# IN2-ViAUn/Exploration-of-Potential

Hardware: AMD Instinct MI355X
Metric: training images/sec, YOLOX-l 24p 640x640 bf16 (higher is better)
Workload: dtype bf16; 1 GPU; YOLOX-l-24p (CSPDarknet53+PAFPN+24p head) train step, 640x640, batch 20/GPU, 10 GTs/img, SimOTA + 24-circle GIoU loss, SGD nesterov; global_batch=20, parallelism=dp1, hip_graph=forward and backward as two lanes of captured segments, loss, update

## Files before the change

exploration-of-potential_amd/csrc/conv_igemm.hip:

```cpp
#include <stdlib.h>
#include <type_traits>
#include <atomic>
#include "igemm.h"

using namespace ep24_igemm;

namespace {

constexpr int KOPT_TILED = 1, KOPT_NARROW_EPI = 2, KOPT_PER_CLASS = 4;
constexpr int KOPT_REMOVED = 16 | 32 | 64;
constexpr int KOPT_NO_DEEP = 128;
constexpr int KOPT_TILED256 = 256;
constexpr int KOPT_NO_WREG = 512;
constexpr int KOPT_PATCH8 = 8;

template <int BN, bool OUT_F32, int EPI, int NSTG = 2>
__device__ __forceinline__ void igemm_dma_tile(const IgemmArgs& p, const int tile_m, const int tile_n) {
    constexpr int WN = BN / 64, WM = 4 / WN, MT = BM / WM / 16, NT = 4;
    constexpr int A_BYTES = BM * 128, B_BYTES = BN * 128, STAGE = A_BYTES + B_BYTES;
    constexpr int A_INSTR = BM * 8 / 64 / 4;
    constexpr int B_INSTR = BN * 8 / 64 / 4;
    extern __shared__ __attribute__((aligned(16))) char smem[];

    const int tid = threadIdx.x, lane = tid & 63, wave = __builtin_amdgcn_readfirstlane(tid >> 6);
// ... 7 lines not shown
    const auto src_rsrc = __builtin_amdgcn_make_buffer_rsrc(const_cast<bf16*>(p.src), 0, p.src_bytes, 0x00020000);
    const auto wt_rsrc = __builtin_amdgcn_make_buffer_rsrc(const_cast<bf16*>(p.wt), 0, p.wt_bytes, 0x00020000);
    int rowoff[A_INSTR];
    unsigned vmask[A_INSTR];
    int iy0v[A_INSTR], ix0v[A_INSTR];
#pragma unroll
    for (int i = 0; i < A_INSTR; ++i) {
        const long m = m0 + (wave * A_INSTR + i) * 8 + (lane >> 3);
        const bool rv = m < p.M;
        const int mm = rv ? (int)m : 0;
        const int n = fdiv(mm, p.d_plane);
        const int rem = mm - n * (p.GH * p.GW);
        const int gy = fdiv(rem, p.d_gw), gx = rem - gy * p.GW;
        const int iy0 = gy * p.sy, ix0 = gx * p.sx;
        rowoff[i] = (int)((((long)n * p.SH * p.SW + (long)iy0 * p.SW + ix0) * p.ld_src + lchunk * 8) * 2);
        iy0v[i] = rv ? iy0 : -(1 << 20);
        ix0v[i] = ix0;
        vmask[i] = 0u;
    }
    const unsigned long long tdy = p.tap_dy, tdx = p.tap_dx, tsl = p.tap_slot;
    for (int t = 0; t < p.T; ++t) {
        const int dy = (int)((tdy >> (4 * t)) & 15ull) - 8, dx = (int)((tdx >> (4 * t)) & 15ull) - 8;
#pragma unroll
        for (int i = 0; i < A_INSTR; ++i) {
            const int iy = iy0v[i] + dy, ix = ix0v[i] + dx;
            if (iy >= 0 && iy < p.SH && ix >= 0 && ix < p.SW) vmask[i] |= 1u << t;
        }
    }
    const int ld2 = (int)p.ld_src * 2;
    int wvoff[B_INSTR];
#pragma unroll
    for (int i = 0; i < B_INSTR; ++i) {
        const int q = (wave * B_INSTR + i) * 8 + (lane >> 3);
        const int r = (q & ~63) + ((q & 15) << 2) + ((q >> 4) & 3);
        wvoff[i] = n0 + r < p.N ? (int)((((long)(n0 + r) * p.WT * p.K) + lchunk * 8) * 2) : OOB;
    }
    const int kmax = (p.K - lchunk * 8 + BK - 1) / BK;
    const int ktail = (p.K & (BK - 1)) ? KC - 1 : KC;

    int is_t = 0, is_kc = 0;
    auto issue = [&](int buf) {
        const int t = is_t, kc = is_kc;
        if (++is_t == p.T) { is_t = 0; ++is_kc; }
        const bool tail = kc >= ktail;
        const int ktm = tail ? -(int)(kc < kmax) : -1;
        const int dy = (int)((tdy >> (4 * t)) & 15ull) - 8, dx = (int)((tdx >> (4 * t)) & 15ull) - 8;
        const int a_s = (dy * p.SW + dx) * ld2 + kc * (BK * 2);
        const unsigned b_s = (unsigned)(((int)((tsl >> (4 * t)) & 15ull) * p.K + kc * BK) * 2);
        char* stage = smem + buf * STAGE;
#pragma unroll
        for (int i = 0; i < A_INSTR; ++i) {
            const int m = -(int)((vmask[i] >> t) & 1u) & ktm;
            const int vo = ((rowoff[i] + a_s) & m) | (OOB & ~m);
            __builtin_amdgcn_raw_ptr_buffer_load_lds(src_rsrc, (lptr_t)(stage + (wave * A_INSTR + i) * 1024), 16, vo, 0, 0, 0);
        }
#pragma unroll
        for (int i = 0; i < B_INSTR; ++i) {
            const int v = (int)((unsigned)wvoff[i] + b_s);
            const int vo = (v & ktm) | (OOB & ~ktm);
            __builtin_amdgcn_raw_ptr_buffer_load_lds(wt_rsrc, (lptr_t)(stage + A_BYTES + (wave * B_INSTR + i) * 1024), 16, vo, 0, 0, 0);
        }
    };

    f32x4 acc[MT][NT];
#pragma unroll
    for (int i = 0; i < MT; ++i)
#pragma unroll
// ... 13 lines not shown
                fb[q] = *reinterpret_cast<const bf16x8*>(lb + swz(wn * 64 + q * 16 + frow, ks * 4 + fq));
#pragma unroll
            for (int i = 0; i < MT; ++i)
#pragma unroll
                for (int q = 0; q < NT; ++q)
                    acc[i][q] = __builtin_amdgcn_mfma_f32_16x16x32_bf16(fa[i], fb[q], acc[i][q], 0, 0, 0);
        }
    };
    if constexpr (NSTG >= 3) {
#pragma unroll
        for (int i = 0; i < NSTG - 1; ++i)
            if (i < n_iter) issue(i);
        int st = 0;
        for (int it = 0; it < n_iter; ++it) {
            const int ahead = n_iter - 1 - it;
            if (NSTG >= 4 && ahead >= 2) asm volatile("s_waitcnt vmcnt(%0)" ::"n"(2 * (A_INSTR + B_INSTR)) : "memory");
            else if (ahead >= 1) asm volatile("s_waitcnt vmcnt(%0)" ::"n"(A_INSTR + B_INSTR) : "memory");
            else asm volatile("s_waitcnt vmcnt(0)" ::: "memory");
            __builtin_amdgcn_s_barrier();
            asm volatile("" ::: "memory");
            if (it + NSTG - 1 < n_iter) issue(st == 0 ? NSTG - 1 : st - 1);
            compute(smem + st * STAGE);
            st = st == NSTG - 1 ? 0 : st + 1;
        }
    } else {
    issue(0);
    for (int it = 0; it < n_iter; ++it) {
        __syncthreads();
        if (it + 1 < n_iter) issue((it + 1) & 1);
        compute(smem + (it & 1) * STAGE);
    }
    }

    igemm_epilogue<BN, OUT_F32, MT, EPI>(p, acc, m0, n0, tile_m, smem);
}

template <int BN, bool OUT_F32, int EPI, int NSTG = 2>
__device__ __forceinline__ void igemm_dma_body(const IgemmArgs& p, const int bid, const int nwg) {
    const int xcd = bid & 7, qq = nwg >> 3, rr = nwg & 7;
    const int tile_id = (xcd < rr ? xcd * (qq + 1) : rr * (qq + 1) + (xcd - rr) * qq) + (bid >> 3);
    const int tiles_n = (p.N + BN - 1) / BN;
    const int tile_m = tile_id / tiles_n;
    igemm_dma_tile<BN, OUT_F32, EPI, NSTG>(p, tile_m, tile_id - tile_m * tiles_n);
}

template <int BN, bool OUT_F32, int EPI = 0>
__global__ __launch_bounds__(256) void igemm_dma_kernel(const IgemmArgs p) {
    igemm_dma_body<BN, OUT_F32, EPI>(p, (int)blockIdx.x, (int)gridDim.x);
}

#ifndef EP24_DEEP_STAGES
#define EP24_DEEP_STAGES 3
#endif
template <int EPI>
__global__ __launch_bounds__(256) void igemm_dma_deep_kernel(const IgemmArgs p) {
    igemm_dma_body<128, false, EPI, EP24_DEEP_STAGES>(p, (int)blockIdx.x, (int)gridDim.x);
}

struct IgemmMulti {
    IgemmArgs a;
    int T[4];
    unsigned long long tap_dy[4], tap_dx[4], tap_slot[4];
    int dy0[4], dx0[4];
    int prefix[5];
    int n;
};

template <int BN>
__global__ __launch_bounds__(256) void igemm_dma_multi_kernel(const IgemmMulti q) {
    int cls = 0;
#pragma unroll
    for (int c = 1; c < 4; ++c)
        if (c < q.n && (int)blockIdx.x >= q.prefix[c]) cls = c;
    cls = __builtin_amdgcn_readfirstlane(cls);
    IgemmArgs p = q.a;
    p.T = q.T[cls];
    p.tap_dy = q.tap_dy[cls]; p.tap_dx = q.tap_dx[cls]; p.tap_slot = q.tap_slot[cls];
    p.dy0 = q.dy0[cls]; p.dx0 = q.dx0[cls];
    igemm_dma_body<BN, false, 1>(p, (int)blockIdx.x - q.prefix[cls], q.prefix[cls + 1] - q.prefix[cls]);
}

template <int BN, int H, int EPI, int NKS, bool ACC, bool GATHER = false, int XF = 0, bool BNR = false>
__global__ __launch_bounds__(256, XF == 3 ? 3 : 2) void igemm_stream_kernel(const IgemmArgs p, int bpn) {
    constexpr int SP = BN / 64, NTW = SP * 4, MT = XF ? 1 : 2, XS = XF ? 2 : 1, RG = 128;
    static_assert(XF == 0 || XF == 4 || H == 1, "the transformed-A forms make one K pass");
    static_assert(!BNR || (EPI == 0 && !GATHER && XF == 4), "the fused reduce belongs to the plain input-gradient form in 16-row blocks (with the transformed-A form it doubled that form's VALU work and spilled: measured, not kept)");
    constexpr int OOB = 0x7FFFFFF0;
    constexpr bool XAUX = XF >= 2;
    constexpr int XNC = XF == 3 ? 5 : XF == 4 ? 0 : 2;
    constexpr int XKP = H * 128;
    constexpr int XC_FLOATS = XF ? XNC * XKP : 0;
    static_assert(XF == 0 || (EPI == 0 && !GATHER), "the transformed-A forms are training forms of the plain 1x1 kernel");
    constexpr int NPAN_ = (H - 1) * 2 + (NKS + 1) / 2;
    extern __shared__ __attribute__((aligned(16))) char smem[];
    const int tid = threadIdx.x, lane = tid & 63, wave = __builtin_amdgcn_readfirstlane(tid >> 6);
    const int frow = lane & 15, fq = lane >> 4;
    const int n_tiles = (p.N + BN - 1) / BN;
    const int xcd = blockIdx.x & 7, rest = blockIdx.x >> 3;
    const int nt = rest % n_tiles, rb = GATHER ? xcd * (bpn >> 3) + rest / n_tiles : (rest / n_tiles) * 8 + xcd;
    const int n0 = nt * BN;

    const auto rsrc = __builtin_amdgcn_make_buffer_rsrc(const_cast<bf16*>(p.src), 0, p.src_bytes, 0x00020000);
    const auto drsrc = __builtin_amdgcn_make_buffer_rsrc(p.dst, 0, p.dst_bytes, 0x00020000);
    const long n_groups = (p.M + RG - 1) / RG;
    const long my_groups = rb < n_groups ? (n_groups - rb + bpn - 1) / bpn : 0;
    const long units = my_groups * H * XS;

    typedef int v4i __attribute__((ext_vector_type(4)));
    typedef unsigned v2u __attribute__((ext_vector_type(2)));
    int gdy[GATHER ? NKS : 1], gdx[GATHER ? NKS : 1], gof[GATHER ? NKS : 1];
    if constexpr (GATHER) {
#pragma unroll
// ... 426 lines not shown
    constexpr int NPAN = (H - 1) * 2 + (NKS + 1) / 2;
    size_t lds = (size_t)NPAN * BN * 128 + (size_t)(XF == 3 ? 5 * H * 128 : (XF == 1 || XF == 2) ? 2 * H * 128 : 0) * sizeof(float) + (size_t)(BNR ? 4 * BN : 0) * sizeof(float);
    if (lds < 4096) lds = 4096;
    const dim3 grid((unsigned)(bpn * n_tiles));
    if constexpr (XF == 3 || BNR) {
        if (a.accumulate) hipLaunchKernelGGL((igemm_stream_kernel<BN, H, 0, NKS, true, false, XF, BNR>), grid, dim3(256), lds, stream, a, (int)bpn);
        else hipLaunchKernelGGL((igemm_stream_kernel<BN, H, 0, NKS, false, false, XF, BNR>), grid, dim3(256), lds, stream, a, (int)bpn);
    } else if constexpr (XF != 0) {
        hipLaunchKernelGGL((igemm_stream_kernel<BN, H, 0, NKS, false, false, XF>), grid, dim3(256), lds, stream, a, (int)bpn);
    } else if constexpr (GATHER) {
        if (a.epi_infer) hipLaunchKernelGGL((igemm_stream_kernel<BN, H, 2, NKS, false, true>), grid, dim3(256), lds, stream, a, (int)bpn);
        else hipLaunchKernelGGL((igemm_stream_kernel<BN, H, 0, NKS, false, true>), grid, dim3(256), lds, stream, a, (int)bpn);
    } else {
        if (a.epi_infer) hipLaunchKernelGGL((igemm_stream_kernel<BN, H, 2, NKS, false>), grid, dim3(256), lds, stream, a, (int)bpn);
        else if (a.accumulate) hipLaunchKernelGGL((igemm_stream_kernel<BN, H, 1, NKS, true>), grid, dim3(256), lds, stream, a, (int)bpn);
        else if (!a.stats) hipLaunchKernelGGL((igemm_stream_kernel<BN, H, 1, NKS, false>), grid, dim3(256), lds, stream, a, (int)bpn);
        else hipLaunchKernelGGL((igemm_stream_kernel<BN, H, 0, NKS, false>), grid, dim3(256), lds, stream, a, (int)bpn);
    }
}

template <int XF>
void launch_stream_xf(const IgemmArgs& a, hipStream_t stream) {
    if (a.N > 64) { if (a.K > 64) launch_stream<128, 1, 4, false, XF>(a, stream); else launch_stream<128, 1, 2, false, XF>(a, stream); }
    else          { if (a.K > 64) launch_stream<64, 1, 4, false, XF>(a, stream); else launch_stream<64, 1, 2, false, XF>(a, stream); }
}

void launch_stream_bnr(const IgemmArgs& a, hipStream_t stream) {
    if (a.N > 64) { if (a.K > 128) launch_stream<128, 2, 4, false, 4, true>(a, stream); else if (a.K > 64) launch_stream<128, 1, 4, false, 4, true>(a, stream); else launch_stream<128, 1, 2, false, 4, true>(a, stream); }
    else          { if (a.K > 128) launch_stream<64, 2, 4, false, 4, true>(a, stream); else if (a.K > 64) launch_stream<64, 1, 4, false, 4, true>(a, stream); else launch_stream<64, 1, 2, false, 4, true>(a, stream); }
}

bool xf_shape_ok(long M, int K, int N) { return K > 0 && K % 8 == 0 && K <= 128 && N > 0 && N % 4 == 0 && N <= 128 && M > 0; }

template <int BN, bool F32>
void launch_variant(const IgemmArgs& a, unsigned tiles, hipStream_t stream) {
    constexpr size_t lds = 2 * (BM * 128 + BN * 128);
    if (a.epi_infer && !F32) hipLaunchKernelGGL((igemm_dma_kernel<BN, false, 2>), dim3(tiles), dim3(256), lds, stream, a);
    else if (!a.stats && !F32) hipLaunchKernelGGL((igemm_dma_kernel<BN, false, 1>), dim3(tiles), dim3(256), lds, stream, a);
    else hipLaunchKernelGGL((igemm_dma_kernel<BN, F32>), dim3(tiles), dim3(256), lds, stream, a);
}

int check_extents(const IgemmArgs& a) {
    for (int t = 0; t < a.T; ++t)
        EP24_REQUIRE(a.T <= 16 && a.oy[t] >= -8 && a.oy[t] <= 7 && a.ox[t] >= -8 && a.ox[t] <= 7 && a.wslot[t] >= 0 && a.wslot[t] <= 15, EP24_E_UNSUPPORTED,
                     "conv: tap %d (offset %d, %d, weight slot %d) does not fit the packed tap tables (offsets -8 .. 7, slots 0 .. 15)", t, a.oy[t], a.ox[t], a.wslot[t]);
    const long src_b = (((long)a.B * a.SH * a.SW - 1) * a.ld_src + a.K) * 2;
    const long wt_b = (long)a.N * a.WT * a.K * 2;
    EP24_REQUIRE(src_b < 0x7FFF0000L && wt_b < 0x7FFF0000L && a.M < (1L << 31) && (long)a.B * a.SH * a.SW < (1L << 31), EP24_E_UNSUPPORTED,
                 "conv: a source of %ld bytes / weights of %ld bytes / %ld output pixels are beyond what the 32-bit tile addressing covers "
                 "(2 GiB per operand): split the batch", src_b, wt_b, (long)a.M);
    return EP24_OK;
}

void prepare(IgemmArgs& a, int kernel_opts) {
    a.narrow_epi = (kernel_opts & KOPT_NARROW_EPI) ? 1 : 0;
    a.src_bytes = (unsigned)((((long)a.B * a.SH * a.SW - 1) * a.ld_src + a.K) * 2);
    a.wt_bytes = (unsigned)((long)a.N * a.WT * a.K * 2);
    a.d_plane = make_fastdiv((unsigned)(a.GH * a.GW)); a.d_gw = make_fastdiv((unsigned)a.GW);
    a.tap_dy = a.tap_dx = a.tap_slot = 0ull;
    for (int t = 0; t < a.T; ++t) {
        a.toff[t] = (int)(((long)a.oy[t] * a.SW + a.ox[t]) * a.ld_src * 2);
        a.tap_dy |= (unsigned long long)((a.oy[t] + 8) & 15) << (4 * t);
        a.tap_dx |= (unsigned long long)((a.ox[t] + 8) & 15) << (4 * t);
        a.tap_slot |= (unsigned long long)(a.wslot[t] & 15) << (4 * t);
    }
}

int launch_multi(IgemmArgs* cls, int n, hipStream_t stream, int kernel_opts) {
    IgemmMulti q{};
    q.n = n;
    bool wide = true;
    for (int i = 0; i < n; ++i) {
        if (int rc = check_extents(cls[i])) return rc;
        prepare(cls[i], kernel_opts);
        {
            const IgemmArgs& c = cls[i];
            const long ext = (((long)(c.B - 1) * c.dbs + c.dp0 + (long)((c.GH - 1) * c.dsy + c.dy0) * c.DW + (c.GW - 1) * c.dsx + c.dx0) * c.ld_dst + c.N) * 2;
            cls[i].dst_bytes = (ext > 0 && ext < 0x7FFF0000L) ? (unsigned)ext : 0u;
        }
        wide = wide && cls[i].N > 64 && (long)ep24_cdiv(cls[i].M, BM) * ep24_cdiv(cls[i].N, 128) > 256;
        const IgemmArgs &x = cls[i], &y = cls[0];
        EP24_REQUIRE(x.src == y.src && x.ld_src == y.ld_src && x.B == y.B && x.SH == y.SH && x.SW == y.SW && x.GH == y.GH && x.GW == y.GW && x.sy == y.sy &&
                     x.sx == y.sx && x.wt == y.wt && x.WT == y.WT && x.K == y.K && x.N == y.N && x.dst == y.dst && x.ld_dst == y.ld_dst && x.DH == y.DH &&
                     x.DW == y.DW && x.dsy == y.dsy && x.dsx == y.dsx && x.dbs == y.dbs && x.dp0 == y.dp0 && x.accumulate == y.accumulate && x.M == y.M &&
                     !x.bias && !x.stats && !x.bnr_z && !x.epi_infer, EP24_E_ARG, "conv_igemm_multi: the classes of one launch share everything but their taps and parity");
    }
    q.a = cls[0];
    for (int i = 1; i < n; ++i) q.a.dst_bytes = (q.a.dst_bytes && cls[i].dst_bytes) ? std::max(q.a.dst_bytes, cls[i].dst_bytes) : 0u;
    for (int i = 0; i < n; ++i) {
        q.T[i] = cls[i].T; q.tap_dy[i] = cls[i].tap_dy; q.tap_dx[i] = cls[i].tap_dx; q.tap_slot[i] = cls[i].tap_slot;
        q.dy0[i] = cls[i].dy0; q.dx0[i] = cls[i].dx0;
        q.prefix[i + 1] = q.prefix[i] + ep24_cdiv(cls[i].M, BM) * ep24_cdiv(cls[i].N, wide ? 128 : 64);
    }
    const unsigned blocks = (unsigned)q.prefix[n];
    const dim3 grid(blocks);
    if (wide) hipLaunchKernelGGL((igemm_dma_multi_kernel<128>), grid, dim3(256), 2 * (BM * 128 + 128 * 128), stream, q);
    else hipLaunchKernelGGL((igemm_dma_multi_kernel<64>), grid, dim3(256), 2 * (BM * 128 + 64 * 128), stream, q);
    EP24_LAUNCH_CHECK("ep24_conv_igemm_multi");
    return EP24_OK;
}

int launch(IgemmArgs a, bool out_f32, hipStream_t stream, int kernel_opts = 0, bool dry = false, int* kernel_id = nullptr) {
    EP24_REQUIRE(!(kernel_opts & KOPT_REMOVED), EP24_E_UNSUPPORTED,
                 "conv: kernel_opts bits 4 - 6 selected variants that were measured, lost and removed; their source is at commit 6cc7180");
    if (!dry) { if (int rc = check_extents(a)) return rc; }
    prepare(a, kernel_opts);
    const bool plain_dst = a.dsy == 1 && a.dsx == 1 && a.dy0 == 0 && a.dx0 == 0 && a.DW == a.GW && a.dp0 == 0 && a.dbs == (long)a.GH * a.GW;
    const long dst_b = ((a.M - 1) * a.ld_dst + a.N) * 2;
    const long dst_ext = plain_dst ? dst_b : (((long)(a.B - 1) * a.dbs + a.dp0 + (long)((a.GH - 1) * a.dsy + a.dy0) * a.DW + (a.GW - 1) * a.dsx + a.dx0) * a.ld_dst + a.N) * 2;
    a.dst_bytes = (!out_f32 && dst_ext > 0 && dst_ext < 0x7FFF0000L) ? (unsigned)dst_ext : 0u;
    const bool stream_ok = a.T == 1 && a.sy == 1 && a.sx == 1 && a.oy[0] == 0 && a.ox[0] == 0 && a.GH == a.SH && a.GW == a.SW &&
                           (a.K <= 128 || (a.K <= 256 && (a.M >= 100000 || !(kernel_opts & KOPT_TILED256)))) && !out_f32 && (!a.bias || a.epi_infer) && plain_dst &&
                           a.ld_dst % 4 == 0 && a.N % 4 == 0 && dst_b < 0x7FFF0000L;
    if (a.bnr_z && !stream_ok) {
        EP24_REQUIRE(plain_dst && !out_f32 && !a.accumulate && !a.narrow_epi && !a.bias && !a.epi_infer && a.N % 8 == 0 && a.ld_dst % 8 == 0 &&
                     a.bnr_ldz % 8 == 0 && ((reinterpret_cast<unsigned long long>(a.dst) | reinterpret_cast<unsigned long long>(a.bnr_z)) & 15) == 0 &&
                     a.bnr_reps > 0, EP24_E_ARG, "conv_dgrad_bnr: needs a plain, first-writer bf16 destination with channel counts / strides in multiples of 8");
    }
    if (stream_ok) {
        if (dry) { *kernel_id = 2; return EP24_OK; }
        a.dst_bytes = (unsigned)dst_b;
        if (a.bnr_z) {
            const long z_b = ((a.M - 1) * a.bnr_ldz + a.N) * 2;
            EP24_REQUIRE(!a.stats && !a.epi_infer && a.bnr_reps > 0 && a.bnr_ldz % 4 == 0 && z_b < 0x7FFF0000L && a.bnr_act == 1, EP24_E_ARG,
                         "conv_dgrad_bnr (1x1): an input gradient of a SiLU unit, z rows 8-byte aligned, operands below 2 GiB");
            a.bnr_z_bytes = (unsigned)z_b;
            launch_stream_bnr(a, stream);
            EP24_LAUNCH_CHECK("ep24_conv_igemm_stream_bnr");
            return EP24_OK;
// ... 7 lines not shown
                            (!a.epi_res || ((a.epi_ldres & 3) == 0 && (reinterpret_cast<unsigned long long>(a.epi_res) & 7) == 0));
    if (a.T == 9 && a.sy == 1 && a.sx == 1 && a.GH == a.SH && a.GW == a.SW && plain_dst && !out_f32 && ((!a.bias && !a.epi_infer) || infer_ring) &&
        !(kernel_opts & KOPT_TILED)) {
        int prc = EP24_OK;
        if (!a.epi_infer && !(kernel_opts & KOPT_NO_WREG) && launch_wreg(a, stream, dry, &prc)) {
            if (dry) { *kernel_id = 6; return EP24_OK; }
            if (prc) return prc;
            EP24_LAUNCH_CHECK("ep24_conv_wreg");
            return EP24_OK;
        }
        if (!(kernel_opts & KOPT_PATCH8) && launch_ring(a, stream, dry, &prc)) {
            if (dry) { *kernel_id = 3; return EP24_OK; }
            if (prc) return prc;
            EP24_LAUNCH_CHECK("ep24_conv_ring");
            return EP24_OK;
        }
        if (!a.epi_infer && launch_patch(a, stream, dry, &prc)) {
            if (dry) { *kernel_id = 1; return EP24_OK; }
            if (prc) return prc;
            EP24_LAUNCH_CHECK("ep24_conv_patch");
            return EP24_OK;
        }
    }
    if (dry) { *kernel_id = 0; return EP24_OK; }
    const bool wide = a.N > 64 && (long)ep24_cdiv(a.M, BM) * ep24_cdiv(a.N, 128) > 256;
    if (!wide && a.N > 64 && !out_f32 && !a.epi_infer && !(kernel_opts & KOPT_NO_DEEP) && a.T * ep24_cdiv(a.K, BK) >= 8) {
        static std::atomic<unsigned long long> done{0};
        int dev = 0;
        EP24_REQUIRE(hipGetDevice(&dev) == hipSuccess, EP24_E_LAUNCH, "conv: hipGetDevice failed");
        const unsigned long long bit = 1ull << (dev & 63);
        if (!(done.load(std::memory_order_acquire) & bit)) {
            hipError_t e = hipFuncSetAttribute((const void*)igemm_dma_deep_kernel<0>, hipFuncAttributeMaxDynamicSharedMemorySize, 160 * 1024);
            if (e == hipSuccess) e = hipFuncSetAttribute((const void*)igemm_dma_deep_kernel<1>, hipFuncAttributeMaxDynamicSharedMemorySize, 160 * 1024);
            EP24_REQUIRE(e == hipSuccess, EP24_E_LAUNCH, "conv: hipFuncSetAttribute(MaxDynamicSharedMemorySize) failed on device %d: %s", dev, hipGetErrorString(e));
            done.fetch_or(bit, std::memory_order_release);
        }
        const unsigned t128 = (unsigned)ep24_cdiv(a.M, BM) * (unsigned)ep24_cdiv(a.N, 128);
        if (a.stats) hipLaunchKernelGGL(igemm_dma_deep_kernel<0>, dim3(t128), dim3(256), EP24_DEEP_STAGES * (BM * 128 + 128 * 128), stream, a);
        else hipLaunchKernelGGL(igemm_dma_deep_kernel<1>, dim3(t128), dim3(256), EP24_DEEP_STAGES * (BM * 128 + 128 * 128), stream, a);
        EP24_LAUNCH_CHECK("ep24_conv_igemm_deep");
        return EP24_OK;
    }
    const unsigned tiles = (unsigned)ep24_cdiv(a.M, BM) * (unsigned)ep24_cdiv(a.N, wide ? 128 : 64);
    if (wide) {
        if (out_f32) launch_variant<128, true>(a, tiles, stream);
        else launch_variant<128, false>(a, tiles, stream);
    } else {
        if (out_f32) launch_variant<64, true>(a, tiles, stream);
        else launch_variant<64, false>(a, tiles, stream);
    }
    EP24_LAUNCH_CHECK("ep24_conv_igemm");
    return EP24_OK;
}

}

static int conv_fwd_impl(const void* x, int64_t ld_x, const void* w, void* y, int64_t ld_y, int y_f32,
                         int64_t y_batch_rows, int64_t y_row0, const float* bias, int64_t* stats,
                         int stats_replicas, int B, int H, int W, int Cin, int Cout, int ksize, int stride,
                         int kernel_opts, void* stream, bool dry = false, int* kernel_id = nullptr) {
    EP24_REQUIRE(dry || (x && w && y), EP24_E_ARG, "conv_fwd: null pointer");
    EP24_REQUIRE(Cin % 8 == 0 && Cin > 0, EP24_E_ARG, "conv_fwd: Cin=%d must be a multiple of 8", Cin);
    EP24_REQUIRE((ksize == 1 || ksize == 3) && (stride == 1 || stride == 2), EP24_E_UNSUPPORTED,
                 "conv_fwd: k=%d s=%d unsupported", ksize, stride);
    EP24_REQUIRE(ld_x % 8 == 0 && (y_f32 || ld_y % 4 == 0), EP24_E_ARG, "conv_fwd: ld_x %% 8 / ld_y %% 4 alignment");
    EP24_REQUIRE(!stats || stats_replicas > 0, EP24_E_ARG, "conv_fwd: stats_replicas");
    const int pad = (ksize - 1) / 2;
    const int OH = (H + 2 * pad - ksize) / stride + 1, OW = (W + 2 * pad - ksize) / stride + 1;
    IgemmArgs a{};
    a.src = (const bf16*)x; a.ld_src = ld_x; a.B = B; a.SH = H; a.SW = W;
    a.GH = OH; a.GW = OW; a.sy = stride; a.sx = stride;
// ... 269 lines not shown
```

exploration-of-potential_amd/csrc/conv_ring.hip:

```cpp
#include <atomic>
#include <type_traits>
#include "igemm.h"

using namespace ep24_igemm;

namespace {

typedef unsigned v4u __attribute__((ext_vector_type(4)));

constexpr int NCW = 4, NLW = 4;
constexpr int NS = 3;
constexpr int RBN = 128, RBM = 256;
constexpr int B_BYTES = RBN * 128;
constexpr int B_INSTR = RBN / 8 / NLW;
constexpr int MT = 8, NT = 4;
constexpr int ZB = 128;
constexpr int LA = 8;
constexpr int SPIN_LIMIT = 1 << 14;

__device__ unsigned g_ring_timeouts;

#ifdef EP24_STAMPS
__device__ unsigned long long g_ring_stamps[64 * 8];
__device__ unsigned long long g_ring_estamps[64 * 8];
// ... 204 lines not shown
__device__ __forceinline__ void ring_store_half(const IgemmArgs& p, long m0, int n0, char* smem) {
    typedef int v4i_ __attribute__((ext_vector_type(4)));
    constexpr int T = ALL ? (NCW + NLW) * 64 : NLW * 64, NK = 4 * 64 * 8 / T;
    const int t = ALL ? (int)threadIdx.x : (int)threadIdx.x - NCW * 64;
    const auto drs = __builtin_amdgcn_make_buffer_rsrc(reinterpret_cast<bf16*>(p.dst), 0, p.dst_bytes, 0x00020000);
    const int rt = t >> 3, ch = t & 7;
    const char* lsrc = smem + HALF * 8192 + rt * 128 + ((ch ^ (rt & 7)) << 4);
    const int ld2 = (int)p.ld_dst * 2;
    const long mt = m0 + HALF * 64 + rt;
    const int cc0 = n0 + ch * 8;
    const int off_t = (int)((mt * p.ld_dst + cc0) * 2);
    bf16x8 v_[NK];
    int off[NK];
#pragma unroll
    for (int k = 0; k < NK; ++k) {
        const int area = ALL ? k : k >> 1, rr = ALL ? 0 : (k & 1) * 32;
        v_[k] = *reinterpret_cast<const bf16x8*>(lsrc + area * 16384 + rr * 128);
        const int dm = (area >> 1) * 128 + rr, dc = (area & 1) * 64;
        off[k] = (mt + dm < p.M && cc0 + dc < p.N) ? off_t + dm * ld2 + dc * 2 : OOB;
    }
    if (p.accumulate) {
        bf16x8 o_[NK];
#pragma unroll
        for (int k = 0; k < NK; ++k) o_[k] = __builtin_bit_cast(bf16x8, __builtin_amdgcn_raw_buffer_load_b128(drs, off[k], 0, 0));
#pragma unroll
        for (int k = 0; k < NK; ++k)
#pragma unroll
            for (int e = 0; e < 8; ++e) v_[k][e] = (bf16)((float)v_[k][e] + (float)o_[k][e]);
    }
#pragma unroll
    for (int k = 0; k < NK; ++k) __builtin_amdgcn_raw_buffer_store_b128(__builtin_bit_cast(v4i_, v_[k]), drs, off[k], 0, 0);
}

template <int PPS, int EMODE>
__global__ __launch_bounds__((NCW + NLW) * 64) void conv_ring_kernel(const IgemmArgs p, const int NP, const int halo, const int npb) {
    extern __shared__ __attribute__((aligned(16))) char smem[];
    const int tid = threadIdx.x, lane = tid & 63, wave = __builtin_amdgcn_readfirstlane(tid >> 6);
    const int nwg = gridDim.x, xcd = blockIdx.x & 7, qq = nwg >> 3, rr = nwg & 7;
    const int tile_id = (xcd < rr ? xcd * (qq + 1) : rr * (qq + 1) + (xcd - rr) * qq) + (blockIdx.x >> 3);
    const int tiles_n = (p.N + RBN - 1) / RBN;
    const int tile_m = tile_id / tiles_n;
    const long m0 = (long)tile_m * RBM;
    const int n0 = (tile_id - tile_m * tiles_n) * RBN;
    const int KC = (p.K + BK - 1) / BK;
    const int PBYTES = NP * 1024;
    const int bb = npb * PBYTES;
    unsigned* const flags = reinterpret_cast<unsigned*>(smem + ZB + bb + NS * B_BYTES);
    lds_u32* const f_full = (lds_u32*)(lptr_t)flags;
    lds_u32* const f_free = f_full + 4;
    lds_u32* const f_err = f_full + 8;
    const int sgn = p.oy[0] < 0 ? 1 : -1;

    if (reinterpret_cast<unsigned long>((lptr_t)smem) != 0ul) {
        if (tid == 0) atomicAdd(&g_ring_timeouts, 1u << 16);
        return;
    }
    if (tid < 12) flags[tid] = 0u;
    if (tid >= 64 && tid < 64 + ZB / 4) reinterpret_cast<unsigned*>(smem)[tid - 64] = 0u;
    __syncthreads();

    const bool wide = !p.narrow_epi && (p.N & 7) == 0 && (p.ld_dst & 7) == 0 && (reinterpret_cast<unsigned long long>(p.dst) & 15) == 0;

    f32x4 acc[MT][NT];
#pragma unroll
    for (int i = 0; i < MT; ++i)
#pragma unroll
        for (int q = 0; q < NT; ++q) acc[i][q] = (f32x4){0.f, 0.f, 0.f, 0.f};
#ifdef EP24_STAMPS
    unsigned long long st_t0 = 0, st_r0 = 0, st_t1 = 0, st_t2 = 0, st_spin = 0;
    unsigned st_nspin = 0;
#endif

    auto loader_main = [&]() {
        const int lw = wave - NCW;
        const int lchunk = (lane & 7) ^ ((lane >> 3) & 7);
        const auto src_rsrc = __builtin_amdgcn_make_buffer_rsrc(const_cast<bf16*>(p.src), 0, p.src_bytes, 0x00020000);
        const auto wt_rsrc = __builtin_amdgcn_make_buffer_rsrc(const_cast<bf16*>(p.wt), 0, p.wt_bytes, 0x00020000);
        const int kmax = (p.K - lchunk * 8 + BK - 1) / BK;
        const int ktail = (p.K & (BK - 1)) ? KC - 1 : KC;
        const int NPW = (NP + NLW - 1) / NLW;
        const unsigned msrc = (unsigned)((long)p.B * p.SH * p.SW);
        const int prow0 = (int)(m0 - halo) + (lane >> 3);
        const int ld2 = (int)p.ld_src * 2;
        const unsigned pv0 = (unsigned)prow0 * (unsigned)ld2 + lchunk * 16;
        auto issue_patch = [&](int pbuf_off, int kc, int i) {
            int g = (i < NPW ? i : NPW - 1) * NLW + lw;
            g = g < NP ? g : NP - 1;
            const unsigned ps = (unsigned)(prow0 + 8 * g);
            bool ok = ps < msrc;
            if (kc >= ktail) ok = ok && kc < kmax;
            const int vo = ok ? (int)(pv0 + (unsigned)(8 * g * ld2 + kc * (BK * 2))) : OOB;
            __builtin_amdgcn_raw_ptr_buffer_load_lds(src_rsrc, (lptr_t)(smem + ZB + pbuf_off + g * 1024), 16, vo, 0, 0, 0);
        };
        int wvoff[B_INSTR];
#pragma unroll
        for (int i = 0; i < B_INSTR; ++i) {
            const int q = (lw * B_INSTR + i) * 8 + (lane >> 3);
            const int r = (q & ~63) + ((q & 15) << 2) + ((q >> 4) & 3);
            wvoff[i] = n0 + r < p.N ? (int)((((long)(n0 + r) * p.WT * p.K) + lchunk * 8) * 2) : OOB;
        }
        auto issue_b = [&](int stage, int t, int kc) {
            const int b_s = (t * p.K + kc * BK) * 2;
#pragma unroll
            for (int i = 0; i < B_INSTR; ++i) {
                int vo = wvoff[i] == OOB ? OOB : wvoff[i] + b_s;
                if (kc >= ktail) vo = kc < kmax ? vo : OOB;
                __builtin_amdgcn_raw_ptr_buffer_load_lds(wt_rsrc, (lptr_t)(smem + ZB + bb + stage * B_BYTES + (lw * B_INSTR + i) * 1024), 16, vo, 0, 0, 0);
            }
        };
        for (int i = 0; i < NPW; ++i) issue_patch(0, 0, i);
        unsigned j = 0;
        for (int kc = 0; kc < KC; ++kc) {
            const int pnext = ((kc + 1) & 1) * PBYTES;
            const bool more = kc + 1 < KC;
#pragma unroll 1
            for (int ty = 0; ty < 3; ++ty) {
                auto step = [&](auto txc) {
                    constexpr int tx = decltype(txc)::value;
                    const int t = ty * 3 + tx;
                    if (j >= (unsigned)NS) spin_until(f_free, j - (NS - 1), f_err);
                    issue_b(tx, t, kc);
                    const bool slice = more && t >= 2;
                    if (slice) {
#pragma unroll
                        for (int i = 0; i < PPS; ++i) issue_patch(pnext, kc + 1, (t - 2) * PPS + i);
                        wait_vmcnt_c<PPS>();
                    } else {
                        wait_vmcnt_c<0>();
                    }
                    ++j;
                    if (lane == 0) st_flag(f_full + lw, j);
// ... 125 lines not shown
                    }
                    if constexpr (g < LA) mma_row(g % MT, pa[g], g < MT ? fb0 : fb1);
                    else mma_row(g % MT, F[g], g < MT ? fb0 : fb1);
                    if constexpr (g >= 9 - LA && g < 9 - LA + MT) {
                        constexpr int i = g - (9 - LA);
                        ra[i] = row_addr(tan, i, tn);
                        pin(ra[i]);
                    }
                    __builtin_amdgcn_sched_barrier(0);
                };
                group(std::integral_constant<int, 0>{}); group(std::integral_constant<int, 1>{});
                group(std::integral_constant<int, 2>{}); group(std::integral_constant<int, 3>{});
                group(std::integral_constant<int, 4>{}); group(std::integral_constant<int, 5>{});
                group(std::integral_constant<int, 6>{}); group(std::integral_constant<int, 7>{});
                group(std::integral_constant<int, 8>{}); group(std::integral_constant<int, 9>{});
                group(std::integral_constant<int, 10>{}); group(std::integral_constant<int, 11>{});
                group(std::integral_constant<int, 12>{}); group(std::integral_constant<int, 13>{});
                group(std::integral_constant<int, 14>{}); group(std::integral_constant<int, 15>{});
                ++j;
            };
            tap_step(std::integral_constant<int, 0>{});
            tap_step(std::integral_constant<int, 1>{});
            tap_step(std::integral_constant<int, 2>{});
        }
    }
#ifdef EP24_STAMPS
    st_t2 = STAMP();
#endif
    };

    const bool consumer = wave < NCW;
    if (consumer) consumer_main(); else loader_main();
    mfma_drain();
    if (wide) ring_epilogue<EMODE>(p, acc, consumer, m0, n0, tile_m, smem);
    else if (consumer) igemm_epilogue<RBN, false, MT, 0, NCW, false>(p, acc, m0, n0, tile_m, smem);
    else return;
    const int cw = wave; (void)cw;
#ifdef EP24_STAMPS
    if (blockIdx.x < 32 && lane == 0 && (cw == 0 || cw == NCW - 1)) {
        unsigned long long* o = g_ring_stamps + (blockIdx.x * 2 + (cw != 0)) * 8;
        o[0] = st_t1 - st_t0; o[1] = st_t2 - st_t1; o[2] = STAMP() - st_t2; o[3] = st_spin; o[4] = st_nspin;
        o[5] = __builtin_amdgcn_s_memrealtime() - st_r0; o[6] = STAMP() - st_t0; o[7] = 9 * KC;
    }
#endif
}

template <int PPS, int EMODE>
int launch_ring_pps(const IgemmArgs& a, int NP, int halo, int npb, size_t lds, hipStream_t stream) {
    const unsigned tiles = (unsigned)ep24_cdiv(a.M, RBM) * (unsigned)ep24_cdiv(a.N, RBN);
    static std::atomic<unsigned long long> done{0};
    int dev = 0;
    EP24_REQUIRE(hipGetDevice(&dev) == hipSuccess, EP24_E_LAUNCH, "conv_ring: hipGetDevice failed");
    const unsigned long long bit = 1ull << (dev & 63);
    if (!(done.load(std::memory_order_acquire) & bit)) {
        const hipError_t e = hipFuncSetAttribute((const void*)conv_ring_kernel<PPS, EMODE>, hipFuncAttributeMaxDynamicSharedMemorySize, 160 * 1024);
        EP24_REQUIRE(e == hipSuccess, EP24_E_LAUNCH, "conv_ring: hipFuncSetAttribute(MaxDynamicSharedMemorySize, 160 KB) failed on device %d: %s", dev,
                     hipGetErrorString(e));
        done.fetch_or(bit, std::memory_order_release);
    }
    IgemmArgs b = a;
    const long dst_b = ((a.M - 1) * a.ld_dst + a.N) * 2;
    EP24_REQUIRE(dst_b < 0x7FFF0000L, EP24_E_UNSUPPORTED, "conv_ring: a destination of %ld bytes is beyond the 32-bit offsets of its stores (launch_ring sends such a layer to the tiled kernel)", dst_b);
    b.dst_bytes = (unsigned)dst_b;
    hipLaunchKernelGGL((conv_ring_kernel<PPS, EMODE>), dim3(tiles), dim3((NCW + NLW) * 64), lds, stream, b, NP, halo, npb);
    return EP24_OK;
}

}

namespace ep24_igemm { int bn_barrier_timeouts(); }

extern "C" int ep24_conv_ring_timeouts(void) {
    unsigned v = 0;
    if (hipMemcpyFromSymbol(&v, HIP_SYMBOL(g_ring_timeouts), sizeof(v)) != hipSuccess) return -1;
    const int bb = ep24_igemm::bn_barrier_timeouts();
    return bb < 0 ? -1 : (int)v + bb;
}

#ifdef EP24_STAMPS
extern "C" int ep24_debug_read_ring_stamps(unsigned long long* host, int n) {
    return hipMemcpyFromSymbol(host, HIP_SYMBOL(g_ring_stamps), sizeof(unsigned long long) * (size_t)n) == hipSuccess ? 0 : -1;
}
extern "C" int ep24_debug_read_ring_estamps(unsigned long long* host, int n) {
    return hipMemcpyFromSymbol(host, HIP_SYMBOL(g_ring_estamps), sizeof(unsigned long long) * (size_t)n) == hipSuccess ? 0 : -1;
}
#endif

namespace ep24_igemm {

bool launch_ring(const IgemmArgs& a, hipStream_t stream, bool dry, int* rc) {
    const int sgn = a.oy[0] < 0 ? 1 : -1;
    for (int t = 0; t < 9; ++t)
        if (a.oy[t] != sgn * (t / 3 - 1) || a.ox[t] != sgn * (t % 3 - 1) || a.wslot[t] != t) return false;
    if (a.K % 8 != 0) return false;
    if (a.bnr_z) return false;
    if (((a.M - 1) * a.ld_dst + a.N) * 2 >= 0x7FFF0000L) return false;
    if (a.N <= 64 || (long)ep24_cdiv(a.M, RBM) * ep24_cdiv(a.N, RBN) < 200) return false;
    const int halo = a.SW + 1;
    const int npb = a.K > BK ? 2 : 1;
    const int np = (RBM + 2 * halo + 7) / 8;
    const size_t lds = ZB + (size_t)npb * np * 1024 + NS * (size_t)B_BYTES + 64;
    const int npw = (np + NLW - 1) / NLW;
    if (lds > 160 * 1024 || npw > 7 * 3) return false;
    if ((size_t)npb * np * 1024 + NS * (size_t)B_BYTES < (size_t)NCW * MT * 16 * 128) return false;
    if (!dry) {
        const int pps = (npw + 6) / 7;
        if (a.epi_infer)
            *rc = pps <= 1 ? launch_ring_pps<1, 1>(a, np, halo, npb, lds, stream)
                : pps == 2 ? launch_ring_pps<2, 1>(a, np, halo, npb, lds, stream)
                           : launch_ring_pps<3, 1>(a, np, halo, npb, lds, stream);
        else if (a.stats)
            *rc = pps <= 1 ? launch_ring_pps<1, 0>(a, np, halo, npb, lds, stream)
                : pps == 2 ? launch_ring_pps<2, 0>(a, np, halo, npb, lds, stream)
                           : launch_ring_pps<3, 0>(a, np, halo, npb, lds, stream);
        else
            *rc = pps <= 1 ? launch_ring_pps<1, 2>(a, np, halo, npb, lds, stream)
                : pps == 2 ? launch_ring_pps<2, 2>(a, np, halo, npb, lds, stream)
                           : launch_ring_pps<3, 2>(a, np, halo, npb, lds, stream);
    }
    return true;
}

}
```

exploration-of-potential_amd/csrc/igemm.h:

```cpp
#pragma once
#include "common.h"

namespace ep24_igemm {

struct IgemmArgs {
    const bf16* src; long ld_src; int B, SH, SW;
    int GH, GW, sy, sx;
    int T; int oy[16]; int ox[16]; int wslot[16];
    const bf16* wt; int WT; int K; int N;
    void* dst; long ld_dst; int DH, DW, dsy, dsx, dy0, dx0; long dbs, dp0;
    int accumulate;
    const float* bias;
    long long* stats; int stats_replicas;
    int epi_act; const bf16* epi_res; long epi_ldres; int epi_infer;
    int toff[16];
    unsigned long long tap_dy, tap_dx, tap_slot;
    unsigned src_bytes, wt_bytes;
    unsigned dst_bytes;
    FastDiv d_plane, d_gw;
    long M;
    int narrow_epi;
    const bf16* bnr_z; long bnr_ldz; const float* bnr_mean; const float* bnr_invstd; const float* bnr_gamma; const float* bnr_beta;
    long long* bnr_dgamma; long long* bnr_dbeta; long bnr_rep_stride; int bnr_reps; int bnr_act;
    unsigned bnr_z_bytes;
// ... 229 lines not shown
        const float bv = fq == 0 ? b4[0] : fq == 1 ? b4[1] : fq == 2 ? b4[2] : b4[3];
        const int c = n0 + wn * 64 + 4 * frow + fq;
        long long* st = p.stats + (long)(tile_m % p.stats_replicas) * 2 * p.N;
        if (c < p.N) {
            atomicAdd((unsigned long long*)(st + c), (unsigned long long)to_fix(av));
            atomicAdd((unsigned long long*)(st + (long)p.N + c), (unsigned long long)to_fix(bv));
        }
    } else if (STATS && p.stats) {
        __syncthreads();
        float* red = reinterpret_cast<float*>(smem);
#pragma unroll
        for (int q = 0; q < 4; ++q) {
            float a = s1[q], b = s2[q];
            a += __shfl_xor(a, 16, 64); a += __shfl_xor(a, 32, 64);
            b += __shfl_xor(b, 16, 64); b += __shfl_xor(b, 32, 64);
            if (fq == 0) {
                red[(wave * 2 + 0) * 64 + 4 * frow + q] = a;
                red[(wave * 2 + 1) * 64 + 4 * frow + q] = b;
            }
        }
        __syncthreads();
        long long* st = p.stats + (long)(tile_m % p.stats_replicas) * 2 * p.N;
        for (int i = tid; i < 2 * BN; i += NWV * 64) {
            const int which = i / BN, c = i - which * BN;
            const int wcol = c >> 6;
            float v = 0.f;
#pragma unroll
            for (int r = 0; r < WM; ++r) v += red[((r * WN + wcol) * 2 + which) * 64 + (c & 63)];
            if (n0 + c < p.N) atomicAdd((unsigned long long*)(st + (long)which * p.N + n0 + c), (unsigned long long)to_fix(v));
        }
    }
}

bool launch_patch(const IgemmArgs& a, hipStream_t stream, bool dry, int* rc);
bool launch_ring(const IgemmArgs& a, hipStream_t stream, bool dry, int* rc);
bool launch_wreg(const IgemmArgs& a, hipStream_t stream, bool dry, int* rc);

}
```

Measured before the change: 1027 images/s.

## Store conv outputs directly from registers by permuting weight rows

After: 1035 images/s (median of 6 runs). About the same (+0.7%).

```diff
diff --git a/exploration-of-potential_amd/csrc/conv_igemm.hip b/exploration-of-potential_amd/csrc/conv_igemm.hip
--- a/exploration-of-potential_amd/csrc/conv_igemm.hip
+++ b/exploration-of-potential_amd/csrc/conv_igemm.hip
@@ -63,7 +63,8 @@
 #pragma unroll
     for (int i = 0; i < B_INSTR; ++i) {
         const int q = (wave * B_INSTR + i) * 8 + (lane >> 3);
-        const int r = (q & ~63) + ((q & 15) << 2) + ((q >> 4) & 3);
+        const int r = EPI == 3 ? (q & ~63) + ((q & 7) << 3) + ((q & 8) >> 1) + ((q >> 4) & 3)
+                               : (q & ~63) + ((q & 15) << 2) + ((q >> 4) & 3);
         wvoff[i] = n0 + r < p.N ? (int)((((long)(n0 + r) * p.WT * p.K) + lchunk * 8) * 2) : OOB;
     }
     const int kmax = (p.K - lchunk * 8 + BK - 1) / BK;
@@ -143,7 +144,8 @@
     }
     }
 
-    igemm_epilogue<BN, OUT_F32, MT, EPI>(p, acc, m0, n0, tile_m, smem);
+    if constexpr (EPI == 3) igemm_store_direct<MT, WN>(p, acc, m0, n0);
+    else igemm_epilogue<BN, OUT_F32, MT, EPI>(p, acc, m0, n0, tile_m, smem);
 }
 
 template <int BN, bool OUT_F32, int EPI, int NSTG = 2>
@@ -177,7 +179,7 @@
     int n;
 };
 
-template <int BN>
+template <int BN, int EPI = 1>
 __global__ __launch_bounds__(256) void igemm_dma_multi_kernel(const IgemmMulti q) {
     int cls = 0;
 #pragma unroll
@@ -188,7 +190,7 @@
     p.T = q.T[cls];
     p.tap_dy = q.tap_dy[cls]; p.tap_dx = q.tap_dx[cls]; p.tap_slot = q.tap_slot[cls];
     p.dy0 = q.dy0[cls]; p.dx0 = q.dx0[cls];
-    igemm_dma_body<BN, false, 1>(p, (int)blockIdx.x - q.prefix[cls], q.prefix[cls + 1] - q.prefix[cls]);
+    igemm_dma_body<BN, false, EPI>(p, (int)blockIdx.x - q.prefix[cls], q.prefix[cls + 1] - q.prefix[cls]);
 }
 
 template <int BN, int H, int EPI, int NKS, bool ACC, bool GATHER = false, int XF = 0, bool BNR = false>
@@ -681,10 +683,16 @@
 
 bool xf_shape_ok(long M, int K, int N) { return K > 0 && K % 8 == 0 && K <= 128 && N > 0 && N % 4 == 0 && N <= 128 && M > 0; }
 
+bool direct_ok(const IgemmArgs& a) {
+    return !a.stats && !a.epi_infer && !a.bias && !a.bnr_z && !a.narrow_epi && a.dst_bytes != 0u && (a.N & 7) == 0 && (a.ld_dst & 7) == 0 &&
+           (reinterpret_cast<unsigned long long>(a.dst) & 15) == 0;
+}
+
 template <int BN, bool F32>
 void launch_variant(const IgemmArgs& a, unsigned tiles, hipStream_t stream) {
     constexpr size_t lds = 2 * (BM * 128 + BN * 128);
-    if (a.epi_infer && !F32) hipLaunchKernelGGL((igemm_dma_kernel<BN, false, 2>), dim3(tiles), dim3(256), lds, stream, a);
+    if (!F32 && direct_ok(a)) hipLaunchKernelGGL((igemm_dma_kernel<BN, false, 3>), dim3(tiles), dim3(256), lds, stream, a);
+    else if (a.epi_infer && !F32) hipLaunchKernelGGL((igemm_dma_kernel<BN, false, 2>), dim3(tiles), dim3(256), lds, stream, a);
     else if (!a.stats && !F32) hipLaunchKernelGGL((igemm_dma_kernel<BN, false, 1>), dim3(tiles), dim3(256), lds, stream, a);
     else hipLaunchKernelGGL((igemm_dma_kernel<BN, F32>), dim3(tiles), dim3(256), lds, stream, a);
 }
@@ -743,7 +751,9 @@
     }
     const unsigned blocks = (unsigned)q.prefix[n];
     const dim3 grid(blocks);
-    if (wide) hipLaunchKernelGGL((igemm_dma_multi_kernel<128>), grid, dim3(256), 2 * (BM * 128 + 128 * 128), stream, q);
+    if (wide && direct_ok(q.a)) hipLaunchKernelGGL((igemm_dma_multi_kernel<128, 3>), grid, dim3(256), 2 * (BM * 128 + 128 * 128), stream, q);
+    else if (wide) hipLaunchKernelGGL((igemm_dma_multi_kernel<128>), grid, dim3(256), 2 * (BM * 128 + 128 * 128), stream, q);
+    else if (direct_ok(q.a)) hipLaunchKernelGGL((igemm_dma_multi_kernel<64, 3>), grid, dim3(256), 2 * (BM * 128 + 64 * 128), stream, q);
     else hipLaunchKernelGGL((igemm_dma_multi_kernel<64>), grid, dim3(256), 2 * (BM * 128 + 64 * 128), stream, q);
     EP24_LAUNCH_CHECK("ep24_conv_igemm_multi");
     return EP24_OK;
@@ -817,11 +827,13 @@
         if (!(done.load(std::memory_order_acquire) & bit)) {
             hipError_t e = hipFuncSetAttribute((const void*)igemm_dma_deep_kernel<0>, hipFuncAttributeMaxDynamicSharedMemorySize, 160 * 1024);
             if (e == hipSuccess) e = hipFuncSetAttribute((const void*)igemm_dma_deep_kernel<1>, hipFuncAttributeMaxDynamicSharedMemorySize, 160 * 1024);
+            if (e == hipSuccess) e = hipFuncSetAttribute((const void*)igemm_dma_deep_kernel<3>, hipFuncAttributeMaxDynamicSharedMemorySize, 160 * 1024);
             EP24_REQUIRE(e == hipSuccess, EP24_E_LAUNCH, "conv: hipFuncSetAttribute(MaxDynamicSharedMemorySize) failed on device %d: %s", dev, hipGetErrorString(e));
             done.fetch_or(bit, std::memory_order_release);
         }
         const unsigned t128 = (unsigned)ep24_cdiv(a.M, BM) * (unsigned)ep24_cdiv(a.N, 128);
         if (a.stats) hipLaunchKernelGGL(igemm_dma_deep_kernel<0>, dim3(t128), dim3(256), EP24_DEEP_STAGES * (BM * 128 + 128 * 128), stream, a);
+        else if (direct_ok(a)) hipLaunchKernelGGL(igemm_dma_deep_kernel<3>, dim3(t128), dim3(256), EP24_DEEP_STAGES * (BM * 128 + 128 * 128), stream, a);
         else hipLaunchKernelGGL(igemm_dma_deep_kernel<1>, dim3(t128), dim3(256), EP24_DEEP_STAGES * (BM * 128 + 128 * 128), stream, a);
         EP24_LAUNCH_CHECK("ep24_conv_igemm_deep");
         return EP24_OK;
diff --git a/exploration-of-potential_amd/csrc/conv_ring.hip b/exploration-of-potential_amd/csrc/conv_ring.hip
--- a/exploration-of-potential_amd/csrc/conv_ring.hip
+++ b/exploration-of-potential_amd/csrc/conv_ring.hip
@@ -260,7 +260,7 @@
     for (int k = 0; k < NK; ++k) __builtin_amdgcn_raw_buffer_store_b128(__builtin_bit_cast(v4i_, v_[k]), drs, off[k], 0, 0);
 }
 
-template <int PPS, int EMODE>
+template <int PPS, int EMODE, bool DIRECT = false>
 __global__ __launch_bounds__((NCW + NLW) * 64) void conv_ring_kernel(const IgemmArgs p, const int NP, const int halo, const int npb) {
     extern __shared__ __attribute__((aligned(16))) char smem[];
     const int tid = threadIdx.x, lane = tid & 63, wave = __builtin_amdgcn_readfirstlane(tid >> 6);
@@ -324,7 +324,8 @@
 #pragma unroll
         for (int i = 0; i < B_INSTR; ++i) {
             const int q = (lw * B_INSTR + i) * 8 + (lane >> 3);
-            const int r = (q & ~63) + ((q & 15) << 2) + ((q >> 4) & 3);
+            const int r = DIRECT ? (q & ~63) + ((q & 7) << 3) + ((q & 8) >> 1) + ((q >> 4) & 3)
+                                 : (q & ~63) + ((q & 15) << 2) + ((q >> 4) & 3);
             wvoff[i] = n0 + r < p.N ? (int)((((long)(n0 + r) * p.WT * p.K) + lchunk * 8) * 2) : OOB;
         }
         auto issue_b = [&](int stage, int t, int kc) {
@@ -516,6 +517,20 @@
     const bool consumer = wave < NCW;
     if (consumer) consumer_main(); else loader_main();
     mfma_drain();
+    if constexpr (DIRECT) {
+        if (!consumer) return;
+#ifdef EP24_STAMPS
+        const unsigned long long e0 = STAMP();
+#endif
+        igemm_store_direct<MT, 2, true>(p, acc, m0, n0);
+#ifdef EP24_STAMPS
+        if (blockIdx.x < 32 && tid == 0) {
+            unsigned long long* o = g_ring_estamps + blockIdx.x * 2 * 8;
+            o[0] = o[1] = o[2] = o[3] = e0; o[4] = o[5] = o[6] = o[7] = STAMP();
+            for (int k = 0; k < 8; ++k) o[8 + k] = 0;
+        }
+#endif
+    } else
     if (wide) ring_epilogue<EMODE>(p, acc, consumer, m0, n0, tile_m, smem);
     else if (consumer) igemm_epilogue<RBN, false, MT, 0, NCW, false>(p, acc, m0, n0, tile_m, smem);
     else return;
@@ -529,7 +544,7 @@
 #endif
 }
 
-template <int PPS, int EMODE>
+template <int PPS, int EMODE, bool DIRECT = false>
 int launch_ring_pps(const IgemmArgs& a, int NP, int halo, int npb, size_t lds, hipStream_t stream) {
     const unsigned tiles = (unsigned)ep24_cdiv(a.M, RBM) * (unsigned)ep24_cdiv(a.N, RBN);
     static std::atomic<unsigned long long> done{0};
@@ -537,7 +552,7 @@
     EP24_REQUIRE(hipGetDevice(&dev) == hipSuccess, EP24_E_LAUNCH, "conv_ring: hipGetDevice failed");
     const unsigned long long bit = 1ull << (dev & 63);
     if (!(done.load(std::memory_order_acquire) & bit)) {
-        const hipError_t e = hipFuncSetAttribute((const void*)conv_ring_kernel<PPS, EMODE>, hipFuncAttributeMaxDynamicSharedMemorySize, 160 * 1024);
+        const hipError_t e = hipFuncSetAttribute((const void*)conv_ring_kernel<PPS, EMODE, DIRECT>, hipFuncAttributeMaxDynamicSharedMemorySize, 160 * 1024);
         EP24_REQUIRE(e == hipSuccess, EP24_E_LAUNCH, "conv_ring: hipFuncSetAttribute(MaxDynamicSharedMemorySize, 160 KB) failed on device %d: %s", dev,
                      hipGetErrorString(e));
         done.fetch_or(bit, std::memory_order_release);
@@ -546,7 +561,7 @@
     const long dst_b = ((a.M - 1) * a.ld_dst + a.N) * 2;
     EP24_REQUIRE(dst_b < 0x7FFF0000L, EP24_E_UNSUPPORTED, "conv_ring: a destination of %ld bytes is beyond the 32-bit offsets of its stores (launch_ring sends such a layer to the tiled kernel)", dst_b);
     b.dst_bytes = (unsigned)dst_b;
-    hipLaunchKernelGGL((conv_ring_kernel<PPS, EMODE>), dim3(tiles), dim3((NCW + NLW) * 64), lds, stream, b, NP, halo, npb);
+    hipLaunchKernelGGL((conv_ring_kernel<PPS, EMODE, DIRECT>), dim3(tiles), dim3((NCW + NLW) * 64), lds, stream, b, NP, halo, npb);
     return EP24_OK;
 }
 
@@ -597,6 +612,10 @@
             *rc = pps <= 1 ? launch_ring_pps<1, 0>(a, np, halo, npb, lds, stream)
                 : pps == 2 ? launch_ring_pps<2, 0>(a, np, halo, npb, lds, stream)
                            : launch_ring_pps<3, 0>(a, np, halo, npb, lds, stream);
+        else if (!a.narrow_epi && (a.N & 7) == 0 && (a.ld_dst & 7) == 0 && (reinterpret_cast<unsigned long long>(a.dst) & 15) == 0)
+            *rc = pps <= 1 ? launch_ring_pps<1, 2, true>(a, np, halo, npb, lds, stream)
+                : pps == 2 ? launch_ring_pps<2, 2, true>(a, np, halo, npb, lds, stream)
+                           : launch_ring_pps<3, 2, true>(a, np, halo, npb, lds, stream);
         else
             *rc = pps <= 1 ? launch_ring_pps<1, 2>(a, np, halo, npb, lds, stream)
                 : pps == 2 ? launch_ring_pps<2, 2>(a, np, halo, npb, lds, stream)
diff --git a/exploration-of-potential_amd/csrc/igemm.h b/exploration-of-potential_amd/csrc/igemm.h
--- a/exploration-of-potential_amd/csrc/igemm.h
+++ b/exploration-of-potential_amd/csrc/igemm.h
@@ -285,6 +285,80 @@
     }
 }
 
+template <int MT, int WN, bool PLAIN = false>
+__device__ __forceinline__ void igemm_store_direct(const IgemmArgs& p, f32x4 (&acc)[MT][4], long m0, int n0) {
+    typedef int v4i_ __attribute__((ext_vector_type(4)));
+    typedef __bf16 bf16x2_ __attribute__((ext_vector_type(2)));
+    const int lane = threadIdx.x & 63, wave = threadIdx.x >> 6;
+    const int wm = wave / WN, wn = wave % WN;
+    const int frow = lane & 15, fq = lane >> 4;
+    const bool fast_dst = (p.dsy == 1 && p.dsx == 1 && p.dy0 == 0 && p.dx0 == 0 && p.DW == p.GW && p.dp0 == 0 &&
+                           p.dbs == (long)p.GH * p.GW);
+    const auto drs = __builtin_amdgcn_make_buffer_rsrc(reinterpret_cast<bf16*>(p.dst), 0, p.dst_bytes, 0x00020000);
+    const int cc = n0 + wn * 64 + (frow & 7) * 8;
+    const int rl = 4 * fq + (frow >> 3);
+    int off_[PLAIN ? 1 : MT][2];
+    if constexpr (!PLAIN) {
+#pragma unroll
+        for (int i = 0; i < MT; ++i)
+#pragma unroll
+            for (int r2 = 0; r2 < 2; ++r2) {
+                const long m = m0 + wm * (MT * 16) + i * 16 + 2 * r2 + rl;
+                long dpix = m;
+                if (!fast_dst) {
+                    const int mm = m < p.M ? (int)m : 0;
+                    const int n = fdiv(mm, p.d_plane);
+                    const int rem = mm - n * (p.GH * p.GW);
+                    const int gy = fdiv(rem, p.d_gw), gx = rem - gy * p.GW;
+                    dpix = (long)n * p.dbs + p.dp0 + (long)(gy * p.dsy + p.dy0) * p.DW + gx * p.dsx + p.dx0;
+                }
+                off_[i][r2] = (m < p.M && cc < p.N) ? (int)((dpix * p.ld_dst + cc) * 2) : OOB;
+            }
+    }
+    const long mw = m0 + wm * (MT * 16) + rl;
+    const int off_w = (int)((mw * p.ld_dst + cc) * 2), ld2 = (int)p.ld_dst * 2;
+    const int live = cc < p.N ? (int)min((long)(MT * 16), p.M - mw) : 0;
+    auto off = [&](int i, int r2) {
+        if constexpr (PLAIN) return i * 16 + 2 * r2 < live ? off_w + (i * 16 + 2 * r2) * ld2 : OOB;
+        else return off_[i][r2];
+    };
+    auto chunk = [&](int i, int r2) {
+        int a[2], b[2];
+#pragma unroll
+        for (int h = 0; h < 2; ++h) {
+            a[h] = __builtin_bit_cast(int, (bf16x2_){(bf16)acc[i][2 * h][2 * r2], (bf16)acc[i][2 * h + 1][2 * r2]});
+            b[h] = __builtin_bit_cast(int, (bf16x2_){(bf16)acc[i][2 * h][2 * r2 + 1], (bf16)acc[i][2 * h + 1][2 * r2 + 1]});
+        }
+        v4i_ v;
+        v[0] = __builtin_amdgcn_update_dpp(a[0], b[0], 0x128, 0xF, 0xC, false);
+        v[1] = __builtin_amdgcn_update_dpp(a[1], b[1], 0x128, 0xF, 0xC, false);
+        v[2] = __builtin_amdgcn_update_dpp(b[0], a[0], 0x128, 0xF, 0x3, false);
+        v[3] = __builtin_amdgcn_update_dpp(b[1], a[1], 0x128, 0xF, 0x3, false);
+        return v;
+    };
+    if (p.accumulate) {
+        bf16x8 o_[MT][2];
+#pragma unroll
+        for (int i = 0; i < MT; ++i)
+#pragma unroll
+            for (int r2 = 0; r2 < 2; ++r2) o_[i][r2] = __builtin_bit_cast(bf16x8, __builtin_amdgcn_raw_buffer_load_b128(drs, off(i, r2), 0, 0));
+#pragma unroll
+        for (int i = 0; i < MT; ++i)
+#pragma unroll
+            for (int r2 = 0; r2 < 2; ++r2) {
+                bf16x8 v = __builtin_bit_cast(bf16x8, chunk(i, r2));
+#pragma unroll
+                for (int e = 0; e < 8; ++e) v[e] = (bf16)((float)v[e] + (float)o_[i][r2][e]);
+                __builtin_amdgcn_raw_buffer_store_b128(__builtin_bit_cast(v4i_, v), drs, off(i, r2), 0, 0);
+            }
+    } else {
+#pragma unroll
+        for (int i = 0; i < MT; ++i)
+#pragma unroll
+            for (int r2 = 0; r2 < 2; ++r2) __builtin_amdgcn_raw_buffer_store_b128(chunk(i, r2), drs, off(i, r2), 0, 0);
+    }
+}
+
 bool launch_patch(const IgemmArgs& a, hipStream_t stream, bool dry, int* rc);
 bool launch_ring(const IgemmArgs& a, hipStream_t stream, bool dry, int* rc);
 bool launch_wreg(const IgemmArgs& a, hipStream_t stream, bool dry, int* rc);
```
